# diff7/tts-king

Hardware: AMD Instinct MI355X
Metric: FS2 train mel-frames/sec/GPU + HiFi-GAN RTF (22.05 kHz), batch=16 (higher is better)
Workload: dtype bf16

## Files before the change

### include/ttsk.h

```cpp
#ifndef TTSK_H
#define TTSK_H

#include <stdint.h>

#ifdef __cplusplus
extern "C" {
#endif

#define TTSK_VERSION 1

#define TTSK_OK 0
#define TTSK_EINVAL (-1)
#define TTSK_ELAUNCH (-2)

int ttsk_version(void);
const char* ttsk_last_error(void);

enum {
  TTSK_GEMM_A_TR      = 1 << 0,
  TTSK_GEMM_B_TR      = 1 << 1,
  TTSK_GEMM_C_F32     = 1 << 2,
  TTSK_GEMM_RELU      = 1 << 3,
  TTSK_GEMM_ADD_R     = 1 << 4,
  TTSK_GEMM_R_F32     = 1 << 5,
// ... 340 lines not shown
                      int accumulate , const int32_t* frame_limit, int seg_len, void* stream);

int ttsk_fs2_loss_nblocks(void);
int ttsk_fs2_loss(const float* mel, const float* post, const float* mel_target, const int64_t* mel_lens, const float* pitch,
                  const float* energy, const float* logd, const float* pitch_target, const float* energy_target,
                  const int64_t* dur_target, const int64_t* src_lens, int B, int T, int T_target, int n_mel, int L,
                  float grad_scale, float* dmel_sum, float* dpost, float* dpitch, float* denergy, float* dlogd,
                  float* partials, float* losses, const int32_t* frame_limit, void* stream);
int ttsk_fs2_loss_mel(const float* mel, const float* post, const float* mel_target, const int64_t* mel_lens, int B, int T, int T_target,
                      int n_mel, float grad_scale, float* dmel_sum, float* dpost, float* partials, const int32_t* frame_limit, void* stream);
int ttsk_fs2_loss_var(const float* pitch, const float* energy, const float* logd, const float* pitch_target, const float* energy_target,
                      const int64_t* dur_target, const int64_t* src_lens, int B, int L, float grad_scale, float* dpitch, float* denergy,
                      float* dlogd, float* partials, void* stream);
int ttsk_fs2_loss_finalize(const float* partials_mel, const float* partials_var, const int64_t* src_lens, int B, int T, int n_mel,
                           const int32_t* frame_limit, float* losses, void* stream);

int ttsk_optim_state_bytes(void);
int ttsk_rng_advance(void* state, void* stream);
int ttsk_dropout_keep_mask(const uint64_t* rng, uint32_t site, int64_t n, float p, uint8_t* keep, void* stream);
typedef struct ttsk_adam_item {
  int64_t off;
  void* pack;
  void* pack_t;
  int32_t Cs, K, Ds, tile0;
} ttsk_adam_item;
int ttsk_optim_step(float* params, float* grads, float* exp_avg, float* exp_avg_sq, void* shadow_bf16, int64_t n, void* state,
                    float* partials, float max_norm, float beta1, float beta2, float eps, int zero_grad, float d_model, float warmup,
                    const float* anneal_steps_host, int n_anneal, float anneal_rate, int advance_rng,
                    const int64_t* dev_ranges, int n_ranges, int64_t range_floats,
                    const ttsk_adam_item* dev_items, int n_items, int n_tiles, const int64_t* dev_gaps, int n_gaps,
// ... 63 lines not shown
```

### tts_king_amd/csrc/batchnorm.hip

```cpp
#include "common.h"

namespace {

struct BnCommon {
  const void* x;
  const float* mean;
  const float* rstd;
  const float* gamma;
  const float* beta;
  const uint64_t* rng;
  int rows, C, use_tanh;
  float p;
  unsigned site;
  int x_f32;
  const int* frame_limit;
  int seg_len;
  uint8_t* keep;
  const long long* lens;
};
__device__ __forceinline__ float tanh_fast(float x) { return 1.f - 2.f * __frcp_rn(__expf(2.f * x) + 1.f); }
__device__ __forceinline__ bool bn_live(const int* frame_limit, int seg_len, int r) {
  return !frame_limit || (r % seg_len) < frame_limit[0];
}
__device__ __forceinline__ int bn_rows(const int* frame_limit, int seg_len, int rows) {
// ... 226 lines not shown
    const f32x4 s1 = *(const f32x4*)(sums + c4), s2 = *(const f32x4*)(sums + a.C + c4);
    float o[4];
#pragma unroll
    for (int e = 0; e < 4; ++e) o[e] = g[e] * rs[e] * (dy[e] - s1[e] * inv_n - xh[e] * s2[e] * inv_n);
    if (!bn_live(a.frame_limit, a.seg_len, r)) o[0] = o[1] = o[2] = o[3] = 0.f;
    *(uint2*)(dx + (int64_t)r * a.C + c4) = make_uint2(pack_bf2(o[0], o[1]), pack_bf2(o[2], o[3]));
  }
}


constexpr int BN_MAX_CHUNKS = 64;
__host__ __device__ inline int bn_slab(int C) { return (C % 64 == 0) ? 64 : C; }

struct BnSlab {
  int c0, slab, tpr, rpi, r_in, cq, rb, re;
  __device__ BnSlab(int C, int rows) {
    slab = bn_slab(C);
    c0 = blockIdx.x * slab;
    tpr = slab >> 2;
    rpi = 256 / tpr;
    r_in = threadIdx.x / tpr;
    cq = threadIdx.x % tpr;
    const int per = (rows + gridDim.y - 1) / gridDim.y;
    rb = blockIdx.y * per;
    re = min(rb + per, rows);
  }
};

__device__ __forceinline__ void bn_slab_store(const BnSlab& g, int C, const float s[4], const float q[4], float* red, float* partials) {
  if (g.r_in < g.rpi) {
#pragma unroll
    for (int e = 0; e < 4; ++e) { red[g.r_in * g.slab + g.cq * 4 + e] = s[e]; red[(g.rpi + g.r_in) * g.slab + g.cq * 4 + e] = q[e]; }
  }
  __syncthreads();
  for (int v = threadIdx.x; v < 2 * g.slab; v += 256) {
    const int half = v >= g.slab, c = v - half * g.slab;
    float acc = 0.f;
    for (int k = 0; k < g.rpi; ++k) acc += red[(half * g.rpi + k) * g.slab + c];
    partials[(int64_t)blockIdx.y * 2 * C + half * C + g.c0 + c] = acc;
  }
}

constexpr int BN_TOT = 256 + 1024;
__device__ __forceinline__ void bn_slab_totals(const float* __restrict__ partials, int nblk, int C, int c0, int slab, double* tot ) {
  const int nq = slab >> 1, groups = 256 / nq;
  const int t = threadIdx.x;
  if (t < groups * nq) {
    const int q = t % nq, g0 = t / nq;
    const int v0 = q * 4;
    const int col = v0 < slab ? c0 + v0 : C + c0 + (v0 - slab);
    double a[4] = {0.0, 0.0, 0.0, 0.0};
    for (int b = g0; b < nblk; b += 16 * groups) {
      f32x4 f[16];
#pragma unroll
      for (int u = 0; u < 16; ++u) {
// ... 183 lines not shown
  if (!act) return;
  const float inv_n = 1.f / bn_rows(a.frame_limit, a.seg_len, a.rows);
  const f32x4 gm = *(const f32x4*)(a.gamma + c4), rsd = *(const f32x4*)(a.rstd + c4);
#pragma unroll
  for (int u = 0; u < 4; ++u) {
    const int r = g.rb + g.r_in + u * g.rpi;
    if (r >= g.re) break;
    float o[4];
#pragma unroll
    for (int e = 0; e < 4; ++e) o[e] = gm[e] * rsd[e] * (dy[u][e] - s1s[cl + e] * inv_n - xh[u][e] * s2s[cl + e] * inv_n);
    if (!bn_live(a.frame_limit, a.seg_len, r)) o[0] = o[1] = o[2] = o[3] = 0.f;
    *(uint2*)(dx + (int64_t)r * a.C + c4) = make_uint2(pack_bf2(o[0], o[1]), pack_bf2(o[2], o[3]));
  }
}

inline int bn_chunks(int rows) { int n = (rows + 15) / 16; return n > BN_MAX_CHUNKS ? BN_MAX_CHUNKS : (n < 1 ? 1 : n); }
inline int bn_apply_chunks(int rows, int C) { const int rpi = 256 / (bn_slab(C) >> 2); int n = (rows + 4 * rpi - 1) / (4 * rpi); return n < 1 ? 1 : n; }

inline int bn_blocks(int rows) { int n = (rows + 15) / 16; return n > 1024 ? 1024 : (n < 1 ? 1 : n); }

}

extern "C" int ttsk_bn_nblocks(int rows) { return bn_blocks(rows); }

static int bn_check(int rows, int C) {
  TTSK_REQUIRE(rows > 0 && C >= 4 && C <= 1024 && (C & 3) == 0, "batchnorm: C must be a multiple of 4, <= 1024 (got %d)", C);
  return 0;
}

static int limit_check(const int32_t* frame_limit, int seg_len, int rows) {
// ... 123 lines not shown
                                   const int32_t* frame_limit, int seg_len, void* stream) {
  if (int rc = limit_check(frame_limit, seg_len, rows)) return rc;
  TTSK_REQUIRE(x && partials && nblk > 0 && mean && rstd && gamma && beta && (out_bf16 || out_f32), "bn_train_apply: null pointer");
  TTSK_REQUIRE((running_mean == nullptr) == (running_var == nullptr), "bn_train_apply: running stats come in pairs");
  TTSK_REQUIRE(p == 0.f || rng, "bn_train_apply: dropout needs rng");
  if (int rc = bn2_check(rows, C)) return rc;
  BnCommon a{x, nullptr, nullptr, gamma, beta, rng, rows, C, use_tanh, p, site, x_is_f32, frame_limit, seg_len > 0 ? seg_len : 1, keep_out};
  BnTrain t{partials, nblk, eps, momentum, mean, rstd, running_mean, running_var, (long long*)num_batches_tracked};
  const dim3 grid(C / bn_slab(C), bn_apply_chunks(rows, C));
  if (resid_f32) hipLaunchKernelGGL(bn_apply2_kernel<true>, grid, dim3(256), 0, (hipStream_t)stream, a, t, resid_f32, (bf16_t*)out_bf16, out_f32);
  else hipLaunchKernelGGL(bn_apply2_kernel<false>, grid, dim3(256), 0, (hipStream_t)stream, a, t, resid_f32, (bf16_t*)out_bf16, out_f32);
  TTSK_CHECK_LAUNCH();
  return TTSK_OK;
}

extern "C" int ttsk_bn_bwd_stats_slab(const void* dout, int dout_is_f32, const void* x, int x_is_f32, const float* mean, const float* rstd,
                                      const float* gamma, const float* beta, int rows, int C, int use_tanh, float p, uint32_t site,
                                      const uint64_t* rng, const uint8_t* keep, float* partials, const int32_t* frame_limit, int seg_len,
                                      void* stream) {
  if (int rc = limit_check(frame_limit, seg_len, rows)) return rc;
  TTSK_REQUIRE(dout && x && mean && rstd && gamma && beta && partials, "bn_bwd_stats_slab: null pointer");
  TTSK_REQUIRE(p == 0.f || rng || keep, "bn_bwd_stats_slab: dropout needs rng or the forward's keep bits");
  if (int rc = bn2_check(rows, C)) return rc;
  BnCommon a{x, mean, rstd, gamma, beta, rng, rows, C, use_tanh, p, site, x_is_f32, frame_limit, seg_len > 0 ? seg_len : 1, (uint8_t*)keep};
  const int slab = bn_slab(C), rpi = 256 / (slab >> 2);
  hipLaunchKernelGGL(bn_bwd_stats2_kernel, dim3(C / slab, bn_chunks(rows)), dim3(256), 2 * rpi * slab * sizeof(float), (hipStream_t)stream,
                     a, dout, dout_is_f32, partials);
  TTSK_CHECK_LAUNCH();
  return TTSK_OK;
}
// ... 17 lines not shown
```

### tts_king_amd/csrc/loss.hip

```cpp
#include "common.h"

namespace {

struct LossArgs {
  const float* mel;
  const float* post;
  const float* mel_t;
  const long long* mel_lens;
  const float* pitch; const float* energy; const float* logd;
  const float* pitch_t; const float* energy_t; const long long* dur_t;
  const long long* src_lens;
  float* dmel_sum;
  float* dpost;
  float* dpitch; float* denergy; float* dlogd;
  float* partials;
  int B, T, Tt, nm, L;
  float grad_scale;
  const int* frame_limit;
};

__device__ __forceinline__ float sgn(float v) { return v > 0.f ? 1.f : (v < 0.f ? -1.f : 0.f); }

template <bool MEL, bool VAR>
__global__ __launch_bounds__(256) void loss_kernel(const LossArgs a) {
  __shared__ float red[6][4];
  const int lane = threadIdx.x & 63, wave = threadIdx.x >> 6;
  float acc[6] = {0, 0, 0, 0, 0, 0};
  const int nm4 = a.nm >> 2;
  const int64_t n4 = (int64_t)a.B * a.T * nm4;
  const float inv_n = 1.f / ((float)a.B * (a.frame_limit ? a.frame_limit[0] : a.T) * a.nm);
  const float gs = a.grad_scale * inv_n;
  if constexpr (MEL)
  for (int64_t i = blockIdx.x * 256 + threadIdx.x; i < n4; i += (int64_t)gridDim.x * 256) {
    const int64_t rt = i / nm4;
    const int c = (int)(i - rt * nm4) * 4;
    const int b = (int)(rt / a.T), t = (int)(rt - (int64_t)b * a.T);
    const bool ok = t < a.mel_lens[b];
    f32x4 dm = {0, 0, 0, 0}, dp = {0, 0, 0, 0};
    if (ok) {
      const f32x4 m = *(const f32x4*)(a.mel + rt * a.nm + c), p = *(const f32x4*)(a.post + rt * a.nm + c);
      const f32x4 tg = *(const f32x4*)(a.mel_t + ((int64_t)b * a.Tt + t) * a.nm + c);
#pragma unroll
      for (int e = 0; e < 4; ++e) {
        const float d1 = m[e] - tg[e], d2 = p[e] - tg[e];
        acc[0] += d1 * d1; acc[1] += fabsf(d1); acc[2] += fabsf(d2);
        dp[e] = gs * sgn(d2);
        dm[e] = gs * (2.f * d1 + sgn(d1)) + dp[e];
      }
    }
    *(f32x4*)(a.dmel_sum + rt * a.nm + c) = dm;
    *(f32x4*)(a.dpost + rt * a.nm + c) = dp;
  }
  if constexpr (VAR) {
  float nv = 0.f;
  for (int b = 0; b < a.B; ++b) nv += (float)a.src_lens[b];
  const float gv = a.grad_scale * 2.f / nv;
  const int nph = a.B * a.L;
  for (int i = blockIdx.x * 256 + threadIdx.x; i < nph; i += gridDim.x * 256) {
    const int b = i / a.L, l = i - b * a.L;
    const bool ok = l < a.src_lens[b];
    float g1 = 0.f, g2 = 0.f, g3 = 0.f;
    if (ok) {
// ... 103 lines not shown
```

### tts_king_amd/fastspeech2.py

```python
import json
import os

import torch
import torch.nn as nn

from . import ops
from . import params as P
from . import switches
from .ops import bf16

N_VOCAB = 207


def sinusoid_table(n_position, d_hid):
    pos = torch.arange(n_position, dtype=torch.float64)[:, None]
    j = torch.arange(d_hid)[None, :]
    angle = pos / torch.pow(torch.tensor(10000.0, dtype=torch.float64), 2.0 * (j // 2).double() / d_hid)
    tab = torch.empty_like(angle)
    tab[:, 0::2] = torch.sin(angle[:, 0::2])
    tab[:, 1::2] = torch.cos(angle[:, 1::2])
    return tab.float()


def get_speakers_number(preprocess_config):
# ... 101 lines not shown
        self._postnet_ends_win = True
        self.dwconv = switches.get("TTSK_DWCONV") != "0"
        self.group_predictors = not self.use_cwt
        self.dw_side_wgs = int(switches.get("TTSK_DW_SIDE_WGS"))
        self.dw_side_frac = float(switches.get("TTSK_DW_SIDE_FRAC"))
        self._dw_side = None
        self._dw_side_pending = False
        self.dp_schedule = switches.get("TTSK_DP_SCHEDULE")
        self._fin_side = None
        self.pred_side = switches.get("TTSK_PRED_SIDE")
        self._pred_stream = None
        self._pred_fwd_pending = False
        self._var_on_pred = False
        self._loss_finalize = None
        self.split_loss = True
        self.grads_partial = False
        self._acc = True
        self._rng_state = None
        self._seed = seed
        self._modules_by_key = {}
        for en in entries:
            self._register(en, device)
        self._init_constants(preprocess_config, model_config)
        self.reset_parameters(seed)
        va = "variance_adaptor."
        o = [self._table[va + n + "_predictor.conv_layer.conv1d_1.conv.weight"].offset for n in ("duration", "pitch", "energy")]
        self._pred_stride = o[1] - o[0]
        if self.use_cwt:
            self._pred_stride = None
            hm = [self._table[va + "pitch_mean." + k].offset for k in
# ... 448 lines not shown
        h1 = torch.empty(3, rows, Fh, dtype=bf16, device=dev)
        ops.conv1d(stack[0].view(Bn, Lp, d), W1, self._m(c + "conv1d_1.conv.bias"), flags=ops.RELU, out=h1[0].view(Bn, Lp, Fh),
                   nz1=3, sA=(rows * d, 0), sB=(ps, 0), sC=(rows * Fh, 0), s_bias1=ps)
        a1, m1, r1, _ = ops.layernorm_fwd_grouped(h1.view(3 * rows, Fh), self._m(c + "layer_norm_1.weight"), self._m(c + "layer_norm_1.bias"),
                                                  3, ps, 2, row_limit, Lp if row_limit is not None else 0, p_post=p, site_post=200, rng=rng)
        h2 = torch.empty(3, rows, Fh, dtype=bf16, device=dev)
        ops.conv1d(a1[:rows].view(Bn, Lp, Fh), W2, self._m(c + "conv1d_2.conv.bias"), flags=ops.RELU, out=h2[0].view(Bn, Lp, Fh),
                   nz1=3, sA=(rows * Fh, 0), sB=(ps, 0), sC=(rows * Fh, 0), s_bias1=ps)
        _, m2, r2, out = ops.layernorm_fwd_grouped(h2.view(3 * rows, Fh), self._m(c + "layer_norm_2.weight"), self._m(c + "layer_norm_2.bias"),
                                                   3, ps, 2, lens, Lp, p_post=p, site_post=201, rng=rng, want_out=False,
                                                   head=(self._m(pre + "linear_layer.weight").view(-1), self._m(pre + "linear_layer.bias")))
        if ctx is not None:
            ctx["grouped"] = (stack, h1, m1, r1, a1, h2, m2, r2, Bn, Lp, lens, p, row_limit)
        return out.view(3, Bn, Lp)

    def _predictors_bwd_grouped(self, saved, dstack, rng, dx3, dxin=None):
        if dxin is None:
            dxin = self._predictors_bwd_inputs(saved, dstack, rng)
        Lp, row_limit = saved[9], saved[12]
        return ops.va_combine(dx3, dxin, Lp, row_limit)

    def _predictors_bwd_inputs(self, saved, dstack, rng, train=True, need_dur_dx=True):
        (stack, h1, m1, r1, a1, h2, m2, r2, Bn, Lp, lens, p, row_limit) = saved
        d, rows, ps = self.d, Bn * Lp, self._pred_stride
        names = ("duration", "pitch", "energy")
        pre = "variance_adaptor.duration_predictor."
        c = pre + "conv_layer."
        W1, W2 = self._w(c + "conv1d_1.conv.weight"), self._w(c + "conv1d_2.conv.weight")
        Fh = W1.shape[0]
        dev = dstack.device
# ... 15 lines not shown
        dh1 = dh1.view(3, rows, Fh)
        for g, n in enumerate(names if train else ()):
            cg = "variance_adaptor.%s_predictor.conv_layer." % n
            self._finalize_ln(part[g], nblk, 3 * Fh, cg + "conv1d_1.conv.bias")
            ops.queue_dw(self._deferred, dh1[g].view(Bn, Lp, Fh), stack[g].view(Bn, Lp, d), self._g(cg + "conv1d_1.conv.weight"), None,
                         self._acc, k=self.k_var, use_dwgemm=self._use_dwconv)
        dxin = torch.empty(3, rows, d, dtype=torch.float32, device=dev)
        if need_dur_dx:
            ops.conv1d_dx(dh1[0].view(Bn, Lp, Fh), W1, out=dxin[0].view(Bn, Lp, d), nz1=3, sA=(rows * Fh, 0), sB=(ps, 0), sC=(rows * d, 0))
        else:
            ops.conv1d_dx(dh1[1].view(Bn, Lp, Fh), self._w("variance_adaptor.pitch_predictor.conv_layer.conv1d_1.conv.weight"),
                          out=dxin[1].view(Bn, Lp, d), nz1=2, sA=(rows * Fh, 0), sB=(ps, 0), sC=(rows * d, 0))
        return dxin

    def _forward(self, train, speakers, texts, src_lens, Lp, mel_lens, max_mel_len, e_targets, d_targets, pitches_raw,
                 p_control, e_control, d_control, frame_limit=None, phoneme_limit=None, defer_pred_join=False):
        if self.use_cwt and phoneme_limit is not None:
            raise ops.L.TtskError("use_cwt: texts padded to a phoneme bucket are not supported (mi355x.l_bucket must be 1)")
        self.sync_shadow()
        dev, d = self.device, self.d
        Bn = texts.shape[0]
        ctx = _Ctx() if train else None
        rng = ops.rng_of(self._state()) if train else None
        p_enc, p_dec, p_var, p_post = (self.p_enc, self.p_dec, self.p_var, self.p_post) if train else (0.0, 0.0, 0.0, 0.0)
        p_pitch = (self.p_pitch if train else 0.0) if self.use_cwt else p_var
        heads = heads_saved = None
        blocks = [] if train else None
        preds = {} if train else None

        grouped = (train and self.group_predictors and pitches_raw is not None and e_targets is not None and Lp <= self.max_seq_len)
        masks_aside = grouped and self.pred_side in ("1", "f") and mel_lens is not None and d_targets is not None and max_mel_len is not None
# ... 75 lines not shown
            nxt = "decoder.layer_stack.%d." % (i + 1) if i + 1 < self.n_dec else None
            y = self._fft_fwd("decoder.layer_stack.%d." % i, y, Bn, T, mlens, self.n_head_dec, p_dec, 100 + 2 * i, rng, blocks, qkv=qkv, next_pre=nxt)
            y, qkv = y if nxt else (y, None)
        rows = Bn * T
        pkm = self._pack("lin", "mel_linear.weight")
        if pkm is not None and y.dtype == bf16:
            mel, mel16 = ops.win_conv_dual(y.view(Bn, T, d), pkm, self.n_mel, 1, bias=self._m("mel_linear.bias"))
            mel, mel16 = mel.view(rows, self.n_mel), mel16.view(rows, self.n_mel)
        else:
            mel16 = torch.empty(rows, self.n_mel, dtype=bf16, device=dev)
            mel = ops.linear(y, self._w("mel_linear.weight"), self._m("mel_linear.bias"), out_dtype=torch.float32, C2=mel16)
        fl = (frame_limit, T) if (frame_limit is not None and train) else None
        if fl is not None:
            ops.zero_frames_from(mel16, fl)
        pn = []
        xin = mel16.view(Bn, T, self.n_mel)
        for i in range(5):
            pp = "postnet.convolutions.%d." % i
            pk = self._pack("pn", pp + "0.conv.weight")
            stats = None
            if pk is not None and xin.dtype == bf16:
                cw = self._table[pp + "0.conv.weight"].storage_shape
                if train and xin.shape[2] in (512, 80) and ops.bn_slab_supported(cw[0]):
                    yc, stats = ops.win_conv_stats(xin, pk, cw[0], cw[1], bias=self._m(pp + "0.conv.bias"), frame_limit=fl)
                else:
                    yc = ops.win_conv(xin, pk, cw[0], cw[1], bias=self._m(pp + "0.conv.bias"), out_dtype=torch.float32)
            else:
                yc = ops.conv1d(xin, self._w(pp + "0.conv.weight"), self._m(pp + "0.conv.bias"), out_dtype=torch.float32)
            C = yc.shape[2]
            last = i == 4
            if train and ops.bn_slab_supported(C):
                nxt, mean, rstd, keep = ops.bn_train(yc.view(rows, C), self.get(pp + "1.running_mean"), self.get(pp + "1.running_var"),
                                                     self.get(pp + "1.num_batches_tracked").view(1), self._m(pp + "1.weight"),
                                                     self._m(pp + "1.bias"), not last, p=p_post, site=300 + i, rng=rng,
                                                     resid=mel if last else None, out_f32=last, frame_limit=fl, want_keep=True,
                                                     partials=stats)
            else:
                keep = None
                if train:
                    mean, rstd = ops.bn_train_stats(yc.view(rows, C), self.get(pp + "1.running_mean"), self.get(pp + "1.running_var"),
                                                    self.get(pp + "1.num_batches_tracked").view(1), frame_limit=fl)
                else:
                    mean, rstd = self.get(pp + "1.running_mean"), ops.rsqrt_eps(self.get(pp + "1.running_var"))
                nxt = ops.bn_apply(yc.view(rows, C), mean, rstd, self._m(pp + "1.weight"), self._m(pp + "1.bias"), not last,
                                   p=p_post, site=300 + i, rng=rng, resid=mel if last else None, out_f32=last, frame_limit=fl)
            pn.append((pp, xin, yc, mean, rstd, keep))
            xin = nxt.view(Bn, T, C) if not last else nxt
        post = xin
        if self._pred_fwd_pending and not defer_pred_join:
            torch.cuda.current_stream().wait_stream(self._pred_stream)
            self._pred_fwd_pending = False
        if train:
            ctx.blocks, ctx.preds, ctx.pn = blocks, preds, pn
            ctx.n_enc_blocks = n_enc_blocks
            ctx.dims = (Bn, Lp, T)
            ctx.texts, ctx.speakers, ctx.pidx, ctx.eidx, ctx.cs = texts, speakers, pidx, eidx, cs
            ctx.dec_out = y
            ctx.frame_limit = fl
            ctx.used = False
            ctx.heads_saved = heads_saved
        out = (mel.view(Bn, T, self.n_mel), pitch, energy, logd, d_rounded, src_masks, mel_masks, mel_lens_out,
               post.view(Bn, T, self.n_mel))
        if self.use_cwt:
            out = out + (heads,)
        return out, ctx

    def _cwt_pitch_rows(self, x1, pitch_cwt, Bn, Lp, p_control):
        va = "variance_adaptor."
        heads, saved = ops.cnnscalar_fwd(x1, pitch_cwt, self._m(va + "pitch_mean.flat_one.net.0.weight", 2 * ops.CNNSCALAR_FLOATS), Bn, Lp)
        self._cwt_head_inputs = (x1, pitch_cwt)
        self._cwt_pitch, pidx = ops.cwt_pitch(pitch_cwt, heads, self.get(va + "pitch_bins"), p_control)
        return pidx, heads, saved

    def eval_front(self, speakers, texts, src_lens, Lp, p_control=1.0, e_control=1.0, d_control=1.0):
        return self._eval_front(speakers, texts, src_lens, Lp, p_control, e_control, d_control, ragged=False)

    def eval_back(self, x3, dur, Lp, T):
# ... 390 lines not shown
        ops.stamp("bwd.start")
        pred_dxin = None
        if self.pred_side in ("1", "b") and "grouped" in ctx.preds and (on_bucket is None or dp_side) and need_below:
            if self._pred_stream is None:
                self._pred_stream = torch.cuda.Stream(device=self.device)
            if not self._var_on_pred:
                self._pred_stream.wait_stream(torch.cuda.current_stream())
            with torch.cuda.stream(self._pred_stream):
                pred_dxin = self._predictors_bwd_inputs(ctx.preds["grouped"], self._stack3(dlogd, dpitch, denergy), rng, **pkw)
        elif self._var_on_pred:
            torch.cuda.current_stream().wait_stream(self._pred_stream)
            self._finalize_loss()
        self._var_on_pred = False
        dout = dpost.view(rows, nm)
        dmel_tot = None
        bn_partials = None
        for i in range(4, -1, -1):
            pp, xin, yc, mean, rstd, keep = ctx.pn[i]
            C = yc.shape[2]
            dy = ops.bn_bwd(dout, yc.view(rows, C), mean, rstd, self._m(pp + "1.weight"), self._m(pp + "1.bias"), i < 4,
                            p=self.p_post, site=300 + i, rng=rng, dgamma=self._g(pp + "1.weight") if pn_on else None,
                            dbeta=self._g(pp + "1.bias") if pn_on else None,
                            frame_limit=ctx.frame_limit, keep=keep, accumulate=self._acc, partials=bn_partials)
            bn_partials = None
            if pn_on:
                ops.colsum_into(dy, self._g(pp + "0.conv.bias"), defer=self._deferred_fin, accumulate=self._acc)
                ops.queue_dw(self._deferred, dy.view(Bn, T, C), xin, self._g(pp + "0.conv.weight"), None, self._acc, k=5,
                             use_dwgemm=self._use_dwconv)
            pkt = self._pack("pnT", pp + "0.conv.weight")
            if i > 0 and pkt is not None:
                cw = self._table[pp + "0.conv.weight"].storage_shape
# ... 95 lines not shown
```

### tts_king_amd/graph.py

```python
import torch

from . import ops


class GraphedTrainStep:

    def __init__(self, enqueue, example_batch, warmup=2, pool=None, static_packed=None, layout=None):
        self.static_packed, self.layout = static_packed, layout
        self.static = list(example_batch) if static_packed is not None else [t.clone() if torch.is_tensor(t) else t for t in example_batch]
        self.graph = torch.cuda.CUDAGraph()
        side = torch.cuda.Stream()
        side.wait_stream(torch.cuda.current_stream())
        with torch.cuda.stream(side):
            for _ in range(warmup):
                enqueue(self.static)
        torch.cuda.current_stream().wait_stream(side)
        torch.cuda.synchronize()
        dist_on = torch.distributed.is_available() and torch.distributed.is_initialized()
        with torch.cuda.graph(self.graph, pool=pool, capture_error_mode="thread_local" if dist_on else "global"):
            self.outputs = enqueue(self.static)

    def key(self):
        return tuple(tuple(t.shape) for t in self.static if torch.is_tensor(t))

# ... 11 lines not shown
                    if torch.is_tensor(dst) and src is not dst:
                        dst.copy_(src, non_blocking=True)
        self.graph.replay()
        return self.outputs


def make_enqueue(model, optimizer, cfg, Loss, step_is_update=True, reducer=None, grad_scale=None, frame_limit=None, phoneme_limit=None,
                 accumulate=None):
    grad_acc = cfg.train_config["optimizer"]["grad_acc_step"]
    gs = (1.0 / grad_acc) if grad_scale is None else grad_scale

    def enqueue(batch):
        dev = model.device
        with torch.no_grad():
            ops.stamp("step.start")
            out, ctx = model._forward(True, batch[2], batch[3], batch[4], int(batch[5]), batch[7], batch[8], batch[9],
                                      batch[10], batch[11], 1.0, 1.0, 1.0, frame_limit=frame_limit, phoneme_limit=phoneme_limit,
                                      defer_pred_join=bool(getattr(model, "split_loss", False)))
            ops.stamp("fwd.done")
            mel, pitch, energy, logd = out[0], out[1], out[2], out[3]
            post = out[8]
            lim = None if frame_limit is None else (frame_limit, 0)
            dh = None
            if getattr(model, "use_cwt", False):
                losses, dmel_sum, dpost, dp, de, dd, dh = ops.fs2_loss_cwt(mel, post, batch[6], batch[7], pitch, out[9], energy, logd, batch[12],
                                                                           batch[13], batch[14], batch[9], batch[10], batch[4], grad_scale=gs,
                                                                           frame_limit=lim)
            elif model._pred_fwd_pending:
                side = model._pred_stream
                losses, dmel_sum, dpost, dp, de, dd, pending = ops.fs2_loss_split(mel, post, batch[6], batch[7], pitch, energy, logd, batch[11], batch[9],
                                                                                  batch[10], batch[4], side, grad_scale=gs, frame_limit=lim)
                model._pred_fwd_pending = False
                model._var_on_pred = True
                model._loss_finalize = lambda: ops.fs2_loss_finalize(losses, pending, batch[4])
            else:
                losses, dmel_sum, dpost, dp, de, dd = ops.fs2_loss(mel, post, batch[6], batch[7], pitch, energy, logd, batch[11],
                                                                   batch[9], batch[10], batch[4], grad_scale=gs, frame_limit=lim)
            if reducer is not None and step_is_update:
                model.backward_native(ctx, dmel_sum, dpost, dp, de, dd, on_bucket=reducer.on_group_done, accumulate=accumulate, dheads=dh)
                reducer.finish()
            else:
                model.backward_native(ctx, dmel_sum, dpost, dp, de, dd, accumulate=accumulate, dheads=dh)
            if step_is_update:
                optimizer.step_and_update_lr(advance_rng=True, keep_grads=True)
            else:
                ops.rng_advance(model._state())
# ... 4 lines not shown
```

### tts_king_amd/ops.py

```python
import ctypes as C

import threading

import torch

from . import lib as L
from .lib import (A_TR, B_TR, C_F32, RELU, ADD_R, R_F32, MASK_G, LRELU_IN, TANH, ACCUM_C, LRELU_OUT, F16, C2_LRELU, DEFER_REDUCE, RAW_SLABS,
                  GemmDesc, check)

bf16 = torch.bfloat16
f16 = torch.float16


def _stream():
    return torch.cuda.current_stream().cuda_stream


def _dev(*ts):
    for t in ts:
        if t is not None and not t.is_cuda:
            raise L.TtskError("tts_king_amd kernels need HIP device tensors (got %s); there is no CPU path" % t.device)


def _ptr(t):
# ... 1305 lines not shown
    Lp = pitch.shape[1]
    dev = mel.device
    lib = L.load()
    dmel, dpost = _f32(B, T, nm, device=dev), _f32(B, T, nm, device=dev)
    dstack = _f32(3, B, Lp, device=dev)
    dd, dp, de = dstack[0], dstack[1], dstack[2]
    partials = _f32(lib.ttsk_fs2_loss_nblocks(), 6, device=dev)
    losses = _f32(8, device=dev)
    check(lib.ttsk_fs2_loss(_ptr(mel), _ptr(post), _ptr(mel_t), _ptr(mel_lens), _ptr(pitch), _ptr(energy), _ptr(logd),
                            _ptr(pitch_t), _ptr(energy_t), _ptr(dur_t), _ptr(src_lens), B, T, Tt, nm, Lp, grad_scale,
                            _ptr(dmel), _ptr(dpost), _ptr(dp), _ptr(de), _ptr(dd), _ptr(partials), _ptr(losses), _lim(frame_limit)[0], _stream()),
          "ttsk_fs2_loss")
    return losses, dmel, dpost, dp, de, dd


def fs2_loss_split(mel, post, mel_t, mel_lens, pitch, energy, logd, pitch_t, energy_t, dur_t, src_lens, side, grad_scale=1.0, frame_limit=None):
    _dev(mel, post, mel_t, mel_lens, pitch, energy, logd, pitch_t, energy_t, dur_t, src_lens)
    B, T, nm = mel.shape
    Tt = mel_t.shape[1]
    Lp = pitch.shape[1]
    dev = mel.device
    lib = L.load()
    dmel, dpost = _f32(B, T, nm, device=dev), _f32(B, T, nm, device=dev)
    partials = _f32(lib.ttsk_fs2_loss_nblocks(), 6, device=dev)
    losses = _f32(8, device=dev)
    lim = _lim(frame_limit)[0]
    check(lib.ttsk_fs2_loss_mel(_ptr(mel), _ptr(post), _ptr(mel_t), _ptr(mel_lens), B, T, Tt, nm, grad_scale, _ptr(dmel), _ptr(dpost), _ptr(partials),
                                lim, _stream()), "ttsk_fs2_loss_mel")
    with torch.cuda.stream(side):
        dstack = _f32(3, B, Lp, device=dev)
        dd, dp, de = dstack[0], dstack[1], dstack[2]
        partials_var = _f32(lib.ttsk_fs2_loss_nblocks(), 6, device=dev)
        check(lib.ttsk_fs2_loss_var(_ptr(pitch), _ptr(energy), _ptr(logd), _ptr(pitch_t), _ptr(energy_t), _ptr(dur_t), _ptr(src_lens), B, Lp,
                                    grad_scale, _ptr(dp), _ptr(de), _ptr(dd), _ptr(partials_var), _stream()), "ttsk_fs2_loss_var")
    return losses, dmel, dpost, dp, de, dd, (partials, partials_var, lim, (B, T, nm))


def fs2_loss_finalize(losses, pending, src_lens):
    partials, partials_var, lim, (B, T, nm) = pending
    check(L.load().ttsk_fs2_loss_finalize(_ptr(partials), _ptr(partials_var), _ptr(src_lens), B, T, nm, lim, _ptr(losses), _stream()),
          "ttsk_fs2_loss_finalize")


# ... 528 lines not shown
```

Before: 2.491 million.

## Fuse PostNet final batchnorm, mel loss and backward stats into one kernel

Adds a postnet_turn kernel that, in a single launch, finalises the last PostNet batchnorm statistics, applies normalise, dropout and the residual mel add, and computes the mel L1/L2 loss terms and their gradients. It also computes the batchnorm backward slab partials that the backward pass later consumes. The aim is to remove separate launches and repeated reads and writes of the mel-sized tensors between the forward batchnorm apply, the loss kernel and the backward stats kernel. In exchange, every block redundantly reduces the stats totals. The path only applies with split loss, no CWT, and one-slab channel counts.

```diff
diff --git a/include/ttsk.h b/include/ttsk.h
--- a/include/ttsk.h
+++ b/include/ttsk.h
@@ -378,6 +378,12 @@
                       float* dlogd, float* partials, void* stream);
 int ttsk_fs2_loss_finalize(const float* partials_mel, const float* partials_var, const int64_t* src_lens, int B, int T, int n_mel,
                            const int32_t* frame_limit, float* losses, void* stream);
+int ttsk_postnet_turn(const void* x, int x_is_f32, const float* stats_partials, int nblk, float eps, float momentum, float* mean,
+                      float* rstd, float* running_mean, float* running_var, int64_t* num_batches_tracked, const float* gamma,
+                      const float* beta, int C, float p, uint32_t site, const uint64_t* rng, const float* mel, float* post,
+                      uint8_t* keep_out, const float* mel_target, const int64_t* mel_lens, int B, int T, int T_target,
+                      float grad_scale, float* dmel_sum, float* dpost, float* loss_partials, float* bwd_partials,
+                      const int32_t* frame_limit, void* stream);
 
 int ttsk_optim_state_bytes(void);
 int ttsk_rng_advance(void* state, void* stream);
diff --git a/tts_king_amd/csrc/batchnorm.hip b/tts_king_amd/csrc/batchnorm.hip
--- a/tts_king_amd/csrc/batchnorm.hip
+++ b/tts_king_amd/csrc/batchnorm.hip
@@ -1,4 +1,5 @@
 #include "common.h"
+#include "loss_terms.h"
 
 namespace {
 
@@ -264,20 +265,21 @@
 
 struct BnSlab {
   int c0, slab, tpr, rpi, r_in, cq, rb, re;
-  __device__ BnSlab(int C, int rows) {
+  __device__ BnSlab(int C, int rows) : BnSlab(C, rows, blockIdx.x, blockIdx.y, gridDim.y) {}
+  __device__ BnSlab(int C, int rows, int bx, int chunk, int nchunks) {
     slab = bn_slab(C);
-    c0 = blockIdx.x * slab;
+    c0 = bx * slab;
     tpr = slab >> 2;
     rpi = 256 / tpr;
     r_in = threadIdx.x / tpr;
     cq = threadIdx.x % tpr;
-    const int per = (rows + gridDim.y - 1) / gridDim.y;
-    rb = blockIdx.y * per;
+    const int per = (rows + nchunks - 1) / nchunks;
+    rb = chunk * per;
     re = min(rb + per, rows);
   }
 };
 
-__device__ __forceinline__ void bn_slab_store(const BnSlab& g, int C, const float s[4], const float q[4], float* red, float* partials) {
+__device__ __forceinline__ void bn_slab_store(const BnSlab& g, int C, const float s[4], const float q[4], float* red, float* partials, int chunk) {
   if (g.r_in < g.rpi) {
 #pragma unroll
     for (int e = 0; e < 4; ++e) { red[g.r_in * g.slab + g.cq * 4 + e] = s[e]; red[(g.rpi + g.r_in) * g.slab + g.cq * 4 + e] = q[e]; }
@@ -287,8 +289,11 @@
     const int half = v >= g.slab, c = v - half * g.slab;
     float acc = 0.f;
     for (int k = 0; k < g.rpi; ++k) acc += red[(half * g.rpi + k) * g.slab + c];
-    partials[(int64_t)blockIdx.y * 2 * C + half * C + g.c0 + c] = acc;
-  }
+    partials[(int64_t)chunk * 2 * C + half * C + g.c0 + c] = acc;
+  }
+}
+__device__ __forceinline__ void bn_slab_store(const BnSlab& g, int C, const float s[4], const float q[4], float* red, float* partials) {
+  bn_slab_store(g, C, s, q, red, partials, blockIdx.y);
 }
 
 constexpr int BN_TOT = 256 + 1024;
@@ -502,6 +507,141 @@
   }
 }
 
+struct TurnLoss {
+  const float* mel_t;
+  const long long* mel_lens;
+  float* dmel_sum;
+  float* dpost;
+  float* partials;
+  float* bwd_partials;
+  int B, T, Tt, n_loss;
+  float grad_scale;
+};
+
+__device__ __forceinline__ unsigned turn_out(const BnCommon& a, const float* ms, const float* rs, int cl, f32x4 gm, f32x4 bt, f32x4 rr, int64_t i,
+                                             unsigned thr, float scale, float v[4]) {
+  unsigned kb = 0xFu;
+#pragma unroll
+  for (int e = 0; e < 4; ++e) v[e] = (v[e] - ms[cl + e]) * rs[cl + e] * gm[e] + bt[e];
+  if (a.p > 0.f) {
+    const uint4 bb = bits4(a.rng, a.site, (unsigned)i);
+    const bool k0 = bb.x >= thr, k1 = bb.y >= thr, k2 = bb.z >= thr, k3 = bb.w >= thr;
+    v[0] = k0 ? v[0] * scale : 0.f; v[1] = k1 ? v[1] * scale : 0.f;
+    v[2] = k2 ? v[2] * scale : 0.f; v[3] = k3 ? v[3] * scale : 0.f;
+    kb = (unsigned)((int)k0 | ((int)k1 << 1) | ((int)k2 << 2) | ((int)k3 << 3));
+  }
+#pragma unroll
+  for (int e = 0; e < 4; ++e) v[e] += rr[e];
+  return kb;
+}
+
+__global__ __launch_bounds__(256) void postnet_turn_kernel(const BnCommon a, const BnTrain t, const float* __restrict__ mel,
+                                                           float* __restrict__ out32, const TurnLoss w) {
+  __shared__ double tot[BN_TOT];
+  __shared__ float ms[128], rs[128];
+  __shared__ float red[2048];
+  const int C = a.C, tid = threadIdx.x;
+  bn_slab_totals(t.partials, t.nblk, C, 0, C, tot);
+  if (tid < C) {
+    const int c = tid;
+    const int n = bn_rows(a.frame_limit, a.seg_len, a.rows);
+    const double m = tot[c] / n;
+    double var = tot[C + c] / n - m * m;
+    if (var < 0.0) var = 0.0;
+    ms[c] = (float)m;
+    rs[c] = (float)(1.0 / sqrt(var + (double)t.eps));
+    if (blockIdx.y == 0) {
+      t.mean[c] = ms[c];
+      t.rstd[c] = rs[c];
+      if (t.run_mean) {
+        t.run_mean[c] = (1.f - t.momentum) * t.run_mean[c] + t.momentum * (float)m;
+        t.run_var[c] = (1.f - t.momentum) * t.run_var[c] + t.momentum * (float)(var * n / (n > 1 ? n - 1 : 1));
+      }
+      if (c == 0 && t.nbt) t.nbt[0] += 1;
+    }
+  }
+  __syncthreads();
+  const unsigned thr = keep_threshold(a.p);
+  const float scale = a.p > 0.f ? 1.f / (1.f - a.p) : 1.f;
+  const int nm4 = C >> 2;
+  const float inv_n = 1.f / ((float)w.B * (a.frame_limit ? a.frame_limit[0] : w.T) * C);
+  const float gs = w.grad_scale * inv_n;
+  if ((int)blockIdx.y < w.n_loss) {
+    const int lane = tid & 63, wave = tid >> 6;
+    float acc[3] = {0.f, 0.f, 0.f};
+    const int64_t n4 = (int64_t)a.rows * nm4;
+    for (int64_t i = blockIdx.y * 256 + tid; i < n4; i += (int64_t)w.n_loss * 256) {
+      const int64_t rt = i / nm4;
+      const int c = (int)(i - rt * nm4) * 4;
+      const int b = (int)(rt / w.T), tt = (int)(rt - (int64_t)b * w.T);
+      float v[4];
+      ldx4(a.x, a.x_f32, rt * C + c, v);
+      const f32x4 m = *(const f32x4*)(mel + rt * C + c);
+      if (bn_live(a.frame_limit, a.seg_len, (int)rt)) {
+        const unsigned kb = turn_out(a, ms, rs, c, *(const f32x4*)(a.gamma + c), *(const f32x4*)(a.beta + c), m, i, thr, scale, v);
+        if (a.keep && a.p > 0.f) a.keep[i] = (uint8_t)kb;
+      } else {
+        v[0] = v[1] = v[2] = v[3] = 0.f;
+        if (a.keep) a.keep[i] = 0;
+      }
+      *(f32x4*)(out32 + rt * C + c) = f32x4{v[0], v[1], v[2], v[3]};
+      f32x4 dm = {0, 0, 0, 0}, dp = {0, 0, 0, 0};
+      if (tt < w.mel_lens[b]) {
+        const f32x4 tg = *(const f32x4*)(w.mel_t + ((int64_t)b * w.Tt + tt) * C + c);
+#pragma unroll
+        for (int e = 0; e < 4; ++e) {
+          float gm, gp;
+          mel_terms(m[e], v[e], tg[e], gs, acc, gm, gp);
+          dm[e] = gm; dp[e] = gp;
+        }
+      }
+      *(f32x4*)(w.dmel_sum + rt * C + c) = dm;
+      *(f32x4*)(w.dpost + rt * C + c) = dp;
+    }
+#pragma unroll
+    for (int q = 0; q < 3; ++q) { const float s = wave_sum(acc[q]); if (lane == 0) red[q * 4 + wave] = s; }
+    __syncthreads();
+    if (tid < 3) w.partials[blockIdx.y * 6 + tid] = red[tid * 4] + red[tid * 4 + 1] + red[tid * 4 + 2] + red[tid * 4 + 3];
+    return;
+  }
+  const BnSlab g(C, a.rows, 0, (int)blockIdx.y - w.n_loss, (int)gridDim.y - w.n_loss);
+  const int c4 = g.cq * 4;
+  float s[4] = {0, 0, 0, 0}, q[4] = {0, 0, 0, 0};
+  if (g.r_in < g.rpi) {
+    const f32x4 gm = *(const f32x4*)(a.gamma + c4), bt = *(const f32x4*)(a.beta + c4);
+    for (int r0 = g.rb + g.r_in; r0 < g.re; r0 += 8 * g.rpi) {
+      float xh[8][4], dy[8][4];
+#pragma unroll
+      for (int u = 0; u < 8; ++u) {
+        const int r = r0 + u * g.rpi, rc = min(r, g.re - 1);
+        const int b = rc / w.T, tt = rc - b * w.T;
+        const int64_t i = (int64_t)rc * nm4 + g.cq;
+        float v[4];
+        ldx4(a.x, a.x_f32, (int64_t)rc * C + c4, v);
+#pragma unroll
+        for (int e = 0; e < 4; ++e) xh[u][e] = (v[e] - ms[c4 + e]) * rs[c4 + e];
+        const f32x4 m = *(const f32x4*)(mel + (int64_t)rc * C + c4);
+        const f32x4 tg = *(const f32x4*)(w.mel_t + ((int64_t)b * w.Tt + tt) * C + c4);
+        const bool live = bn_live(a.frame_limit, a.seg_len, rc);
+        const unsigned kb = turn_out(a, ms, rs, c4, gm, bt, m, i, thr, scale, v);
+        const bool ok = tt < w.mel_lens[b];
+#pragma unroll
+        for (int e = 0; e < 4; ++e) {
+          float d = ok ? mel_dpost(v[e], tg[e], gs) : 0.f;
+          if (a.p > 0.f) d = ((kb >> e) & 1u) ? d * scale : 0.f;
+          dy[u][e] = d;
+        }
+        if (!live || r >= g.re) { xh[u][0] = xh[u][1] = xh[u][2] = xh[u][3] = 0.f; dy[u][0] = dy[u][1] = dy[u][2] = dy[u][3] = 0.f; }
+      }
+#pragma unroll
+      for (int u = 0; u < 8; ++u)
+#pragma unroll
+        for (int e = 0; e < 4; ++e) { s[e] += dy[u][e]; q[e] += dy[u][e] * xh[u][e]; }
+    }
+  }
+  bn_slab_store(g, C, s, q, red, w.bwd_partials, (int)blockIdx.y - w.n_loss);
+}
+
 inline int bn_chunks(int rows) { int n = (rows + 15) / 16; return n > BN_MAX_CHUNKS ? BN_MAX_CHUNKS : (n < 1 ? 1 : n); }
 inline int bn_apply_chunks(int rows, int C) { const int rpi = 256 / (bn_slab(C) >> 2); int n = (rows + 4 * rpi - 1) / (4 * rpi); return n < 1 ? 1 : n; }
 
@@ -655,6 +795,29 @@
   return TTSK_OK;
 }
 
+extern "C" int ttsk_postnet_turn(const void* x, int x_is_f32, const float* stats_partials, int nblk, float eps, float momentum, float* mean,
+                                 float* rstd, float* running_mean, float* running_var, int64_t* num_batches_tracked, const float* gamma,
+                                 const float* beta, int C, float p, uint32_t site, const uint64_t* rng, const float* mel, float* post,
+                                 uint8_t* keep_out, const float* mel_target, const int64_t* mel_lens, int B, int T, int T_target,
+                                 float grad_scale, float* dmel_sum, float* dpost, float* loss_partials, float* bwd_partials,
+                                 const int32_t* frame_limit, void* stream) {
+  TTSK_REQUIRE(x && stats_partials && nblk > 0 && mean && rstd && gamma && beta && mel && post && mel_target && mel_lens && dmel_sum &&
+                   dpost && loss_partials && bwd_partials, "postnet_turn: null pointer");
+  TTSK_REQUIRE(B > 0 && T > 0 && T_target >= T && (int64_t)B * T < (1ll << 31), "postnet_turn: bad sizes B=%d T=%d T_target=%d", B, T, T_target);
+  TTSK_REQUIRE((running_mean == nullptr) == (running_var == nullptr), "postnet_turn: running stats come in pairs");
+  TTSK_REQUIRE(p == 0.f || (rng && keep_out), "postnet_turn: dropout needs rng and a keep buffer");
+  const int rows = B * T;
+  if (int rc = bn2_check(rows, C)) return rc;
+  TTSK_REQUIRE(bn_slab(C) == C, "postnet_turn: one channel slab only (C = 64, or <= 128 and no multiple of 64; got %d)", C);
+  BnCommon a{x, nullptr, nullptr, gamma, beta, rng, rows, C, 0, p, site, x_is_f32, frame_limit, T, keep_out};
+  BnTrain t{stats_partials, nblk, eps, momentum, mean, rstd, running_mean, running_var, (long long*)num_batches_tracked};
+  const int n_loss = ttsk_fs2_loss_nblocks();
+  TurnLoss w{mel_target, (const long long*)mel_lens, dmel_sum, dpost, loss_partials, bwd_partials, B, T, T_target, n_loss, grad_scale};
+  hipLaunchKernelGGL(postnet_turn_kernel, dim3(1, n_loss + bn_chunks(rows)), dim3(256), 0, (hipStream_t)stream, a, t, mel, post, w);
+  TTSK_CHECK_LAUNCH();
+  return TTSK_OK;
+}
+
 extern "C" int ttsk_bn_bwd_stats_slab(const void* dout, int dout_is_f32, const void* x, int x_is_f32, const float* mean, const float* rstd,
                                       const float* gamma, const float* beta, int rows, int C, int use_tanh, float p, uint32_t site,
                                       const uint64_t* rng, const uint8_t* keep, float* partials, const int32_t* frame_limit, int seg_len,
diff --git a/tts_king_amd/csrc/loss.hip b/tts_king_amd/csrc/loss.hip
--- a/tts_king_amd/csrc/loss.hip
+++ b/tts_king_amd/csrc/loss.hip
@@ -1,4 +1,5 @@
 #include "common.h"
+#include "loss_terms.h"
 
 namespace {
 
@@ -18,8 +19,6 @@
   float grad_scale;
   const int* frame_limit;
 };
-
-__device__ __forceinline__ float sgn(float v) { return v > 0.f ? 1.f : (v < 0.f ? -1.f : 0.f); }
 
 template <bool MEL, bool VAR>
 __global__ __launch_bounds__(256) void loss_kernel(const LossArgs a) {
@@ -42,10 +41,9 @@
       const f32x4 tg = *(const f32x4*)(a.mel_t + ((int64_t)b * a.Tt + t) * a.nm + c);
 #pragma unroll
       for (int e = 0; e < 4; ++e) {
-        const float d1 = m[e] - tg[e], d2 = p[e] - tg[e];
-        acc[0] += d1 * d1; acc[1] += fabsf(d1); acc[2] += fabsf(d2);
-        dp[e] = gs * sgn(d2);
-        dm[e] = gs * (2.f * d1 + sgn(d1)) + dp[e];
+        float gm, gp;
+        mel_terms(m[e], p[e], tg[e], gs, acc, gm, gp);
+        dm[e] = gm; dp[e] = gp;
       }
     }
     *(f32x4*)(a.dmel_sum + rt * a.nm + c) = dm;
diff --git a/tts_king_amd/csrc/loss_terms.h b/tts_king_amd/csrc/loss_terms.h
--- /dev/null
+++ b/tts_king_amd/csrc/loss_terms.h
@@ -0,0 +1,13 @@
+#pragma once
+#include "common.h"
+
+__device__ __forceinline__ float sgn(float v) { return v > 0.f ? 1.f : (v < 0.f ? -1.f : 0.f); }
+
+__device__ __forceinline__ float mel_dpost(float p, float tg, float gs) { return gs * sgn(p - tg); }
+
+__device__ __forceinline__ void mel_terms(float m, float p, float tg, float gs, float* acc, float& dm, float& dp) {
+  const float d1 = m - tg, d2 = p - tg;
+  acc[0] += d1 * d1; acc[1] += fabsf(d1); acc[2] += fabsf(d2);
+  dp = gs * sgn(d2);
+  dm = gs * (2.f * d1 + sgn(d1)) + dp;
+}
diff --git a/tts_king_amd/fastspeech2.py b/tts_king_amd/fastspeech2.py
--- a/tts_king_amd/fastspeech2.py
+++ b/tts_king_amd/fastspeech2.py
@@ -139,6 +139,7 @@
         self._var_on_pred = False
         self._loss_finalize = None
         self.split_loss = True
+        self.fused_turns = True
         self.grads_partial = False
         self._acc = True
         self._rng_state = None
@@ -617,6 +618,19 @@
             ctx["grouped"] = (stack, h1, m1, r1, a1, h2, m2, r2, Bn, Lp, lens, p, row_limit)
         return out.view(3, Bn, Lp)
 
+    def postnet_turn(self, ctx, mel_t, mel_lens, grad_scale=1.0):
+        pp, yc, stats, mel, fl, p_post = ctx.post_turn
+        Bn, _, T = ctx.dims
+        C = yc.shape[2]
+        post, mean, rstd, keep, dmel_sum, dpost, partials, bwd_partials = ops.postnet_turn(
+            yc.view(Bn * T, C), stats, self.get(pp + "1.running_mean"), self.get(pp + "1.running_var"),
+            self.get(pp + "1.num_batches_tracked").view(1), self._m(pp + "1.weight"), self._m(pp + "1.bias"), mel, mel_t, mel_lens, Bn,
+            p=p_post, site=304, rng=ops.rng_of(self._state()), grad_scale=grad_scale, frame_limit=fl)
+        ctx.pn[4] = ctx.pn[4][:3] + (mean, rstd, keep)
+        ctx.bn_partials_last = bwd_partials
+        ctx.post_turn = None
+        return post.view(Bn, T, C), (dmel_sum, dpost, partials)
+
     def _predictors_bwd_grouped(self, saved, dstack, rng, dx3, dxin=None):
         if dxin is None:
             dxin = self._predictors_bwd_inputs(saved, dstack, rng)
@@ -662,7 +676,7 @@
         return dxin
 
     def _forward(self, train, speakers, texts, src_lens, Lp, mel_lens, max_mel_len, e_targets, d_targets, pitches_raw,
-                 p_control, e_control, d_control, frame_limit=None, phoneme_limit=None, defer_pred_join=False):
+                 p_control, e_control, d_control, frame_limit=None, phoneme_limit=None, defer_pred_join=False, defer_post_turn=False):
         if self.use_cwt and phoneme_limit is not None:
             raise ops.L.TtskError("use_cwt: texts padded to a phoneme bucket are not supported (mi355x.l_bucket must be 1)")
         self.sync_shadow()
@@ -768,6 +782,7 @@
         if fl is not None:
             ops.zero_frames_from(mel16, fl)
         pn = []
+        post_turn = None
         xin = mel16.view(Bn, T, self.n_mel)
         for i in range(5):
             pp = "postnet.convolutions.%d." % i
@@ -783,6 +798,11 @@
                 yc = ops.conv1d(xin, self._w(pp + "0.conv.weight"), self._m(pp + "0.conv.bias"), out_dtype=torch.float32)
             C = yc.shape[2]
             last = i == 4
+            if last and train and defer_post_turn and self._pred_fwd_pending and ops.postnet_turn_supported(C):
+                post_turn = (pp, yc, stats, mel, fl, p_post)
+                pn.append((pp, xin, yc, None, None, None))
+                xin = None
+                break
             if train and ops.bn_slab_supported(C):
                 nxt, mean, rstd, keep = ops.bn_train(yc.view(rows, C), self.get(pp + "1.running_mean"), self.get(pp + "1.running_var"),
                                                      self.get(pp + "1.num_batches_tracked").view(1), self._m(pp + "1.weight"),
@@ -813,8 +833,10 @@
             ctx.frame_limit = fl
             ctx.used = False
             ctx.heads_saved = heads_saved
+            ctx.post_turn = post_turn
+            ctx.bn_partials_last = None
         out = (mel.view(Bn, T, self.n_mel), pitch, energy, logd, d_rounded, src_masks, mel_masks, mel_lens_out,
-               post.view(Bn, T, self.n_mel))
+               post.view(Bn, T, self.n_mel) if post is not None else None)
         if self.use_cwt:
             out = out + (heads,)
         return out, ctx
@@ -1235,7 +1257,9 @@
         self._var_on_pred = False
         dout = dpost.view(rows, nm)
         dmel_tot = None
-        bn_partials = None
+        if ctx.post_turn is not None:
+            raise RuntimeError("the forward left the PostNet's last normalise to postnet_turn(ctx, ...), which was not called")
+        bn_partials = ctx.bn_partials_last
         for i in range(4, -1, -1):
             pp, xin, yc, mean, rstd, keep = ctx.pn[i]
             C = yc.shape[2]
diff --git a/tts_king_amd/graph.py b/tts_king_amd/graph.py
--- a/tts_king_amd/graph.py
+++ b/tts_king_amd/graph.py
@@ -49,12 +49,17 @@
         dev = model.device
         with torch.no_grad():
             ops.stamp("step.start")
+            split = bool(getattr(model, "split_loss", False))
             out, ctx = model._forward(True, batch[2], batch[3], batch[4], int(batch[5]), batch[7], batch[8], batch[9],
                                       batch[10], batch[11], 1.0, 1.0, 1.0, frame_limit=frame_limit, phoneme_limit=phoneme_limit,
-                                      defer_pred_join=bool(getattr(model, "split_loss", False)))
-            ops.stamp("fwd.done")
+                                      defer_pred_join=split, defer_post_turn=split and not getattr(model, "use_cwt", False) and bool(getattr(model, "fused_turns", False)))
             mel, pitch, energy, logd = out[0], out[1], out[2], out[3]
             post = out[8]
+            mel_done = None
+            if ctx.post_turn is not None:
+                post, mel_done = model.postnet_turn(ctx, batch[6], batch[7], grad_scale=gs)
+                out = out[:8] + (post,) + out[9:]
+            ops.stamp("fwd.done")
             lim = None if frame_limit is None else (frame_limit, 0)
             dh = None
             if getattr(model, "use_cwt", False):
@@ -64,7 +69,8 @@
             elif model._pred_fwd_pending:
                 side = model._pred_stream
                 losses, dmel_sum, dpost, dp, de, dd, pending = ops.fs2_loss_split(mel, post, batch[6], batch[7], pitch, energy, logd, batch[11], batch[9],
-                                                                                  batch[10], batch[4], side, grad_scale=gs, frame_limit=lim)
+                                                                                  batch[10], batch[4], side, grad_scale=gs, frame_limit=lim,
+                                                                                  mel_done=mel_done)
                 model._pred_fwd_pending = False
                 model._var_on_pred = True
                 model._loss_finalize = lambda: ops.fs2_loss_finalize(losses, pending, batch[4])
diff --git a/tts_king_amd/ops.py b/tts_king_amd/ops.py
--- a/tts_king_amd/ops.py
+++ b/tts_king_amd/ops.py
@@ -1343,19 +1343,55 @@
     return losses, dmel, dpost, dp, de, dd
 
 
-def fs2_loss_split(mel, post, mel_t, mel_lens, pitch, energy, logd, pitch_t, energy_t, dur_t, src_lens, side, grad_scale=1.0, frame_limit=None):
+def postnet_turn(x, stats_partials, running_mean, running_var, nbt, gamma, beta, mel, mel_t, mel_lens, Bn, p=0.0, site=0, rng=None,
+                 grad_scale=1.0, frame_limit=None, eps=1e-5, momentum=0.1):
+    _dev(x, mel, mel_t, mel_lens)
+    rows, Cn = x.shape
+    T = rows // Bn
+    dev = x.device
+    lib = L.load()
+    lp, seg = _lim(frame_limit)
+    if rows != Bn * T or tuple(mel.shape) != (rows, Cn) or mel.dtype != torch.float32 or mel_t.shape[0] != Bn or mel_t.shape[2] != Cn \
+            or not mel_t.is_contiguous() or (frame_limit is not None and seg != T):
+        raise L.TtskError("postnet_turn: x %s, mel %s %s, target %s, B = %d" % (tuple(x.shape), tuple(mel.shape), mel.dtype, tuple(mel_t.shape), Bn))
+    xf = int(x.dtype == torch.float32)
+    if stats_partials is None:
+        stats_partials = _f32(lib.ttsk_bn_nchunks(rows), 2 * Cn, device=dev)
+        check(lib.ttsk_bn_stats_slab(_ptr(x), xf, rows, Cn, _ptr(stats_partials), lp, seg, _stream()), "ttsk_bn_stats_slab")
+    mean, rstd = _f32(Cn, device=dev), _f32(Cn, device=dev)
+    post = _f32(rows, Cn, device=dev)
+    keep = torch.empty(rows, Cn // 4, dtype=torch.uint8, device=dev) if p > 0.0 else None
+    dmel, dpost = _f32(Bn, T, Cn, device=dev), _f32(Bn, T, Cn, device=dev)
+    partials = _f32(lib.ttsk_fs2_loss_nblocks(), 6, device=dev)
+    bwd_partials = _f32(lib.ttsk_bn_nchunks(rows), 2 * Cn, device=dev)
+    check(lib.ttsk_postnet_turn(_ptr(x), xf, _ptr(stats_partials), stats_partials.shape[0], eps, momentum, _ptr(mean), _ptr(rstd),
+                                _ptr(running_mean), _ptr(running_var), _ptr(nbt), _ptr(gamma), _ptr(beta), Cn, p, site, _ptr(rng), _ptr(mel),
+                                _ptr(post), _ptr(keep), _ptr(mel_t), _ptr(mel_lens), Bn, T, mel_t.shape[1], grad_scale, _ptr(dmel), _ptr(dpost),
+                                _ptr(partials), _ptr(bwd_partials), lp, _stream()), "ttsk_postnet_turn")
+    return post, mean, rstd, keep, dmel, dpost, partials, bwd_partials
+
+
+def postnet_turn_supported(Cn):
+    return bn_slab_supported(Cn) and (Cn == 64 or Cn % 64 != 0)
+
+
+def fs2_loss_split(mel, post, mel_t, mel_lens, pitch, energy, logd, pitch_t, energy_t, dur_t, src_lens, side, grad_scale=1.0, frame_limit=None,
+                   mel_done=None):
     _dev(mel, post, mel_t, mel_lens, pitch, energy, logd, pitch_t, energy_t, dur_t, src_lens)
     B, T, nm = mel.shape
     Tt = mel_t.shape[1]
     Lp = pitch.shape[1]
     dev = mel.device
     lib = L.load()
-    dmel, dpost = _f32(B, T, nm, device=dev), _f32(B, T, nm, device=dev)
-    partials = _f32(lib.ttsk_fs2_loss_nblocks(), 6, device=dev)
     losses = _f32(8, device=dev)
     lim = _lim(frame_limit)[0]
-    check(lib.ttsk_fs2_loss_mel(_ptr(mel), _ptr(post), _ptr(mel_t), _ptr(mel_lens), B, T, Tt, nm, grad_scale, _ptr(dmel), _ptr(dpost), _ptr(partials),
-                                lim, _stream()), "ttsk_fs2_loss_mel")
+    if mel_done is not None:
+        dmel, dpost, partials = mel_done
+    else:
+        dmel, dpost = _f32(B, T, nm, device=dev), _f32(B, T, nm, device=dev)
+        partials = _f32(lib.ttsk_fs2_loss_nblocks(), 6, device=dev)
+        check(lib.ttsk_fs2_loss_mel(_ptr(mel), _ptr(post), _ptr(mel_t), _ptr(mel_lens), B, T, Tt, nm, grad_scale, _ptr(dmel), _ptr(dpost), _ptr(partials),
+                                    lim, _stream()), "ttsk_fs2_loss_mel")
     with torch.cuda.stream(side):
         dstack = _f32(3, B, Lp, device=dev)
         dd, dp, de = dstack[0], dstack[1], dstack[2]
```

Result: no change. 2.507 million (median of 6 runs) (+0.7%).
